# ucl-medical-genomics/hygeia

Hardware: AMD Instinct MI355X
Metric: CpG sites/sec through forward-backward; 28M CpG, K=6, 2 seeds, 1/2/4/8 GPUs (higher is better)
Workload: dtype f64; 1 GPU; C3 two_group 28000000 CpG (22 chromosomes, 100k segments + 5k buffers), 4+4 samples, K=6, M=50, B=25, 2 seeds in total, chains sharded over the GPUs (LPT); chains_per_rank=582, threads_per_chain=256, chains_per_cu_resident=3, global_sites_x_seeds=56000000, parallelism=chains over 1 rank(s) on 1 GPU(s)

## Files before the change

### hygeia_amd/_lib.py

```python
from __future__ import annotations

import ctypes as C
import math
import os

KMAX = 16
HERE = os.path.dirname(os.path.abspath(__file__))
LIB_PATH = os.path.join(HERE, "lib", "libhygeia_amd.so")

HYG_OK, HYG_EINVAL, HYG_ENUMERIC, HYG_EDEVICE, HYG_ENOMEM, HYG_EUNSUPPORTED = 0, -1, -2, -3, -4, -5
ERROR_NAMES = {0: "HYG_OK", -1: "HYG_EINVAL", -2: "HYG_ENUMERIC", -3: "HYG_EDEVICE", -4: "HYG_ENOMEM",
               -5: "HYG_EUNSUPPORTED"}


class HygError(RuntimeError):
    def __init__(self, code: int, msg: str):
        super().__init__(f"{ERROR_NAMES.get(code, code)}: {msg}")
        self.code = code


class TgParams(C.Structure):
    _fields_ = [
        ("n_regimes", C.c_int32),
        ("minimum_duration", C.c_int32),
# ... 70 lines not shown
        ("use_adam", C.c_int32),
        ("normalise_gradients", C.c_int32),
        ("n_steps_without_update", C.c_int32),
        ("_pad", C.c_int32),
        ("learning_rate_exponent", C.c_double),
        ("learning_rate_factor", C.c_double),
    ]


class SgChain(C.Structure):
    _fields_ = [
        ("site_begin", C.c_int64),
        ("n_sites", C.c_int32),
        ("_pad", C.c_int32),
        ("seed", C.c_uint64),
        ("chain_id", C.c_uint64),
        ("out_begin", C.c_int64),
    ]


EXPORTS = ("hyg_tg_params_default", "hyg_tg_model_create", "hyg_tg_model_destroy", "hyg_tg_num_particles",
           "hyg_tg_global_weights", "hyg_tg_backward_threads_per_chain", "hyg_tg_kernel_name",
           "hyg_tg_threads_per_chain", "hyg_tg_force_threads", "hyg_tg_set_tail_overlap", "hyg_tg_set_gather_window",
           "hyg_tg_device_cus",
           "hyg_tg_set_device_cus", "hyg_sg_force_key_drop", "hyg_tg_chains_per_cu", "hyg_tg_lds_bytes",
           "hyg_tg_emission", "hyg_tg_workspace_bytes", "hyg_tg_run_chains", "hyg_tg_run_chain_host",
           "hyg_tg_run_chains_host", "hyg_tg_models_compatible", "hyg_tg_workspace_bytes_multi",
           "hyg_tg_run_chains_multi", "hyg_tg_run_chains_host_multi", "hyg_tg_kernel_name_multi",
           "hyg_tg_filter_workspace_bytes", "hyg_tg_filter_workspace_bytes_multi", "hyg_tg_filter_chains",
           "hyg_tg_filter_chains_multi", "hyg_tg_filter_chains_host", "hyg_tg_filter_chains_host_multi",
           "hyg_tg_filter_kernel_name", "hyg_tg_filter_kernel_name_multi",
           "hyg_tg_trace_chains", "hyg_tg_trace_chains_multi", "hyg_tg_trace_chains_host",
           "hyg_tg_trace_chains_host_multi", "hyg_tg_trace_kernel_name", "hyg_tg_trace_kernel_name_multi",
           "hyg_device_count", "hyg_device_slot_acquire", "hyg_device_slot_release", "hyg_set_device",
           "hyg_get_device", "hyg_last_error", "hyg_version", "hyg_set_kernel_timing", "hyg_tg_last_kernel_ms",
           "hyg_sg_params_default", "hyg_sg_model_create", "hyg_sg_model_destroy", "hyg_sg_emission",
           "hyg_sg_workspace_bytes", "hyg_sg_run_chains", "hyg_sg_run_chain_host",
           "hyg_sg_pe_params_default", "hyg_sg_pe_theta_rows", "hyg_sg_pe_workspace_bytes", "hyg_sg_run_chains_pe",
           "hyg_sg_run_chain_host_pe", "hyg_sg_models_compatible", "hyg_sg_workspace_bytes_multi",
           "hyg_sg_pe_workspace_bytes_multi", "hyg_sg_run_chains_multi", "hyg_sg_run_chains_pe_multi",
           "hyg_sg_run_chains_host_multi", "hyg_bed_labels", "hyg_bed_format", "hyg_pre_collapse",
           "hyg_dmp_site_counts", "hyg_dmp_fdr", "hyg_dmp_weighted_fdr", "hyg_tg_posterior_counts")


class DmpGroup(C.Structure):

# ... 28 lines not shown
        _build.build()
    L = C.CDLL(path)
    vp, i32, i64, u64, sz = C.c_void_p, C.c_int32, C.c_int64, C.c_uint64, C.c_size_t
    L.hyg_tg_params_default.restype = None
    L.hyg_tg_params_default.argtypes = [C.POINTER(TgParams)]
    L.hyg_tg_model_create.restype = C.c_int
    L.hyg_tg_model_create.argtypes = [C.POINTER(TgParams), i32, i32, C.POINTER(vp)]
    L.hyg_tg_model_destroy.restype = None
    L.hyg_tg_model_destroy.argtypes = [vp]
    L.hyg_tg_num_particles.restype = i32
    L.hyg_tg_num_particles.argtypes = [vp]
    L.hyg_tg_global_weights.restype = i32
    L.hyg_tg_global_weights.argtypes = [vp]
    L.hyg_tg_threads_per_chain.restype = i32
    L.hyg_tg_threads_per_chain.argtypes = [vp, i32]
    L.hyg_tg_backward_threads_per_chain.restype = i32
    L.hyg_tg_backward_threads_per_chain.argtypes = [vp, i32]
    L.hyg_tg_force_threads.restype = C.c_int
    L.hyg_tg_force_threads.argtypes = [i32, i32]
    L.hyg_tg_set_tail_overlap.restype = C.c_int
    L.hyg_tg_set_tail_overlap.argtypes = [i32]
    L.hyg_tg_set_gather_window.restype = C.c_int
    L.hyg_tg_set_gather_window.argtypes = [i32]
    L.hyg_tg_device_cus.restype = i32
    L.hyg_tg_device_cus.argtypes = [i32]
    L.hyg_tg_set_device_cus.restype = C.c_int
    L.hyg_tg_set_device_cus.argtypes = [i32, i32]
    L.hyg_sg_force_key_drop.restype = C.c_int
    L.hyg_sg_force_key_drop.argtypes = [i32]
    L.hyg_tg_chains_per_cu.restype = i32
    L.hyg_tg_chains_per_cu.argtypes = [vp, i32]
    L.hyg_tg_lds_bytes.restype = sz
    L.hyg_tg_lds_bytes.argtypes = [vp, i32, i32]
    L.hyg_tg_kernel_name.restype = i32
    L.hyg_tg_kernel_name.argtypes = [vp, i32, i32, C.c_char_p, i32]
    L.hyg_tg_emission.restype = C.c_int
    L.hyg_tg_emission.argtypes = [vp, vp, vp, i32, vp, vp, i32, i64, vp, vp]
    L.hyg_tg_workspace_bytes.restype = sz
    L.hyg_tg_workspace_bytes.argtypes = [vp, i32, i64]
    L.hyg_tg_run_chains.restype = C.c_int
    L.hyg_tg_run_chains.argtypes = [vp, C.POINTER(TgChain), i32, vp, vp, sz, C.POINTER(TgOutputs), vp]
    L.hyg_tg_run_chain_host.restype = C.c_int
    L.hyg_tg_run_chain_host.argtypes = [vp, vp, vp, i32, vp, vp, i32, i32, u64, u64, vp, vp, vp, vp, vp, vp, vp]
    L.hyg_tg_run_chains_host.restype = C.c_int
    L.hyg_tg_run_chains_host.argtypes = [vp, vp, vp, i32, vp, vp, i32, i64, C.POINTER(TgChain), i32, i64,
                                         vp, vp, vp, vp, vp, vp, vp, vp]
# ... 162 lines not shown
```

### hygeia_amd/csrc/capi.cpp

```cpp
#include <hip/hip_runtime.h>
#include <fcntl.h>
#include <sys/file.h>
#include <unistd.h>

#include <algorithm>
#include <cerrno>
#include <cmath>
#include <cstdio>
#include <cstring>
#include <map>
#include <memory>
#include <mutex>
#include <string>
#include <vector>

#include "../../include/hyg_arith.h"
#include "../../include/hygeia_amd.h"
#include "../../include/hyg_sg_model.h"
#include "sg_common.h"
#include "tg_common.h"
#include "dmp_common.h"

namespace hyg {
int bed_launch_labels(const double* probs, int K, int64_t n, int8_t* label, double* score, void* stream);
// ... 365 lines not shown
int32_t hyg_tg_kernel_name(const hyg_tg_model* m, int32_t n_chains, int32_t backward, char* buf, int32_t len) {
  if (!m || len < 0) return fail(HYG_EINVAL, "null model or negative length");
  const char* name = nullptr;
  if (hyg::tg_kernel_name(m->c, n_chains, backward != 0, &name) != HYG_OK) return fail_unsupported_shape(m);
  const int32_t need = (int32_t)std::strlen(name) + 1;
  if (buf && len > 0) std::snprintf(buf, (size_t)len, "%s", name);
  return need;
}

int hyg_tg_force_threads(int32_t forward, int32_t backward) {
  const int rc = hyg::tg_force_threads(forward, backward);
  return rc == HYG_OK ? rc : fail(rc, "unsupported workgroup size");
}

int hyg_tg_set_tail_overlap(int32_t on) {
  hyg::tg_set_tail_overlap(on != 0);
  return HYG_OK;
}

int hyg_tg_set_gather_window(int32_t positions) {
  const int rc = hyg::tg_set_gather_window(positions);
  return rc == HYG_OK ? rc : fail(rc, "gather window out of [-1, 256]");
}

int32_t hyg_tg_device_cus(int32_t device) { return hyg::tg_device_cus(device); }

int hyg_tg_set_device_cus(int32_t device, int32_t cus) {
  const int rc = hyg::tg_set_device_cus(device, cus);
  return rc == HYG_OK ? rc : fail(rc, "device out of [0, 64) or negative CU count");
}

int hyg_sg_force_key_drop(int32_t bits) {
  const int rc = hyg::sg_force_key_drop(bits);
  return rc == HYG_OK ? rc : fail(rc, "key bits out of range [8, 60]");
}

int hyg_tg_emission(const hyg_tg_model* m, const uint16_t* meth_c, const uint16_t* tot_c, int32_t s_c,
                    const uint16_t* meth_k, const uint16_t* tot_k, int32_t s_k, int64_t n_sites, double* E,
                    void* stream) {
  if (!m) return fail(HYG_EINVAL, "null model");
  if (!m->on_device) return fail(HYG_EDEVICE, "no HIP device: hygeia_amd has no CPU fallback");
  if (!on_model_device(m->device)) return fail(HYG_EINVAL, "the current HIP device is not the model's device");
  if (s_c < 0 || s_k < 0 || n_sites < 0) return fail(HYG_EINVAL, "negative size");
  if (n_sites > 0 && (!E || (s_c && (!meth_c || !tot_c)) || (s_k && (!meth_k || !tot_k))))
    return fail(HYG_EINVAL, "null buffer");
  return launch_emission(m->dev(), m->c, meth_c, tot_c, s_c, meth_k, tot_k, s_k, n_sites, E, stream);
// ... 1408 lines not shown
```

### hygeia_amd/csrc/tg_common.h

```cpp
#pragma once

#include <stddef.h>
#include <stdint.h>

#include "../../include/hyg_model.h"

namespace hyg {

constexpr int kDefaultThreads = 256;
constexpr int kDefaultThreadsBwd = 256;
constexpr int kLowOccThreads = 512;
constexpr int kLowOccThreadsBwd = 768;
constexpr int kEBlock = 8;

struct ChainDev {
  int64_t site_begin;
  int64_t out_begin;
  int64_t ws_offset;
  uint64_t seed;
  uint64_t chain_id;
  int32_t T;
  int32_t pad;
  int64_t wg_offset;
};
// ... 35 lines not shown
int launch_chains_multi(const ModelDev* models_dev, const hyg_tg_consts& c, const ChainDev* chains_dev, int n_chains,
                        const double* E, uint8_t* ws, const hyg_tg_outputs& out, void* stream);
int launch_filter(const ModelDev& md, const hyg_tg_consts& c, const ChainDev* chains_dev, int n_chains,
                  const double* E, uint8_t* ws, const hyg_tg_outputs& out, void* stream);
int launch_filter_multi(const ModelDev* models_dev, const hyg_tg_consts& c, const ChainDev* chains_dev, int n_chains,
                        const double* E, uint8_t* ws, const hyg_tg_outputs& out, void* stream);
int launch_trace(const ModelDev& md, const hyg_tg_consts& c, const ChainDev* chains_dev, int n_chains, const double* E,
                 uint8_t* ws, const hyg_tg_outputs& out, const hyg_tg_trace& trace, void* stream);
int launch_trace_multi(const ModelDev* models_dev, const hyg_tg_consts& c, const ChainDev* chains_dev, int n_chains,
                       const double* E, uint8_t* ws, const hyg_tg_outputs& out, const hyg_tg_trace& trace,
                       void* stream);
void set_kernel_timing(bool on);
int last_kernel_ms(float* out3);
int tg_threads_per_chain(const hyg_tg_consts& c, int n_chains);
int tg_threads_per_chain_bwd(const hyg_tg_consts& c, int n_chains);
int tg_kernel_name(const hyg_tg_consts& c, int n_chains, bool backward, const char** name, bool multi = false);
int tg_filter_kernel_name(const hyg_tg_consts& c, int n_chains, const char** name, bool multi = false);
int tg_trace_kernel_name(const hyg_tg_consts& c, int n_chains, const char** name, bool multi = false);
size_t tg_trace_lds_bytes(const hyg_tg_consts& c, int n_chains);
int tg_force_threads(int fwd, int bwd);
int tg_resident_per_cu(const hyg_tg_consts& c, int n_chains);
void tg_set_tail_overlap(bool on);
int tg_set_gather_window(int positions);
int tg_device_cus(int dev);
int tg_set_device_cus(int dev, int cus);
size_t tg_layout_bytes(const hyg_tg_consts& c, int threads, bool backward);
bool backward_global_w(const hyg_tg_consts& c);
bool forward_global_w(const hyg_tg_consts& c);
size_t chain_scratch_bytes(const hyg_tg_consts& c);

}
```

### hygeia_amd/csrc/tg_kernels.hip

```cpp
#include <hip/hip_runtime.h>

#include <cstdio>
#include <cstdlib>
#include <atomic>
#include <mutex>
#include <vector>

#include "../../include/hyg_arith.h"
#include "tg_common.h"
#include "hyg_dev.h"

namespace hyg {

enum { MODE_KEEP = 0, MODE_OPTIMAL = 1, MODE_UNBIASED = 2, MODE_INIT = 3 };

#ifndef HYG_SERIAL_PRIO
#define HYG_SERIAL_PRIO 1
#endif
__device__ __forceinline__ void serial_begin() {
  if constexpr (HYG_SERIAL_PRIO > 0) __builtin_amdgcn_s_setprio(HYG_SERIAL_PRIO);
}
__device__ __forceinline__ void serial_end() {
  if constexpr (HYG_SERIAL_PRIO > 0) __builtin_amdgcn_s_setprio(0);
}


__device__ __forceinline__ uint64_t sort_key(float x, int idx) {
  uint32_t u = hyg_f32_bits(x);
  if (u == 0x80000000u) u = 0;
  const uint32_t ord = (u >> 31) ? ~u : (u | 0x80000000u);
  return ((uint64_t)(~ord) << 32) | (uint32_t)idx;
}
__device__ __forceinline__ float key_value(uint64_t k) {
  const uint32_t ord = ~(uint32_t)(k >> 32);
  const uint32_t u = (ord & 0x80000000u) ? (ord & 0x7fffffffu) : ~ord;
  return hyg_bits_f32(u);
}
__device__ __forceinline__ int key_index(uint64_t k) { return (int)(uint32_t)k; }

__device__ __forceinline__ int fdiv(int n, int d, float rd) {
  int q = (int)((float)n * rd);
  if (q * d > n) --q;
  if ((q + 1) * d <= n) ++q;
  return q;
}

template <int R>
// ... 208 lines not shown
#endif
#ifndef HYG_LR512
#define HYG_LR512 2
#endif
template <int NT>
constexpr int kLRof = NT >= 768 ? 2 : (NT >= 512 ? HYG_LR512 : HYG_LR256);
#ifndef HYG_SORT_WAVES
#define HYG_SORT_WAVES 4
#endif
#ifndef HYG_TSF1
#define HYG_TSF1 1
#endif
template <int NT>
constexpr int kSortWaves = (NT / 64 < HYG_SORT_WAVES) ? NT / 64 : HYG_SORT_WAVES;

struct Lay {
  uint32_t W, L, keys, bcnt, bpos, pre64, part, cp, pst, pw, phz, pf, ering, cl, parents, X, grp, gst, rb, xo, red,
      sh, uring, total;
  uint32_t bcnt_bytes;
  int npad, nkeys, nt;
  int topset_r;
  int lcap;
  int gather_w;
};

__host__ __device__ constexpr int bwd_list_doubles(int NT) {
  return (64 * 16 + 128 + 32) > 4 * (NT + 1) ? (64 * 16 + 128 + 32) : 4 * (NT + 1);
}

__host__ __device__ inline size_t fwd_keys_bytes(int Nmax, int NT) {
  size_t kb = sizeof(uint64_t) * (size_t)Nmax;
  if (kb < sizeof(hyg_u128) * (size_t)(NT + 1)) kb = sizeof(hyg_u128) * (size_t)(NT + 1);
  return kb;
}
__host__ __device__ inline size_t fwd_scratch_bytes(int Nmax, int NT) {
  return align_up(sizeof(double) * (size_t)Nmax, 16) + fwd_keys_bytes(Nmax, NT);
}

__host__ __device__ inline Lay make_layout(int K, int M, int B, int Nmax, int NT, bool backward, bool gw = false) {
  Lay l{};
  l.nt = NT;
  l.topset_r = 1;
  l.npad = Nmax;
  l.lcap = (backward && gw && bwd_list_doubles(NT) < Nmax) ? bwd_list_doubles(NT) : Nmax;
  size_t o = 0;
  if (!backward && gw) {
// ... 604 lines not shown
    for (int step = 32; step >= 1; step >>= 1) {
#pragma unroll
      for (int r = 0; r < NSW; ++r) pos[r] += (buf[64 * r + pos[r] + step - 1] < e) ? step : 0;
    }
    int rank = 0;
#pragma unroll
    for (int r = 0; r < NSW; ++r) rank += pos[r] + ((buf[64 * r + pos[r]] < e) ? 1 : 0);
    buf[64 * NSW + rank] = e;
  }
  lds_barrier();
  return sorter ? buf[64 * NSW + base] : e;
}

constexpr int bitonic_lds_stages(int n, int R) {
  int c = 0;
  for (int kk = 2; kk <= n; kk *= 2)
    for (int j = kk / 2; j >= 1; j /= 2) c += (j >= 64 * R) ? 1 : 0;
  return c;
}

template <int NT, int NSW, int R>
__device__ __forceinline__ int top_set_finish(uint64_t* srt, int nA, bool hasB, int N, int M, int cnt_fin, const hyg_u192& massB,
                              unsigned char* scr, int* parents, Shared& sh, const ConstLds& cl, unsigned char* red,
                              float Usys, unsigned long long* ph, bool timed) {
  static_assert(NSW <= NT / 64, "sorting waves");
  const int lane = lane_id();
  const bool sorter = (NSW == NT / 64) || wave_id() < NSW;
  const int base = (int)(threadIdx.x >> 6) * 64 * R + lane * R;
  uint64_t e[R];
  hyg_u192 f[R];
  hyg_u192 loc = hyg_u192_zero();
  if (sorter) {
#pragma unroll
    for (int r = 0; r < R; ++r) e[r] = (base + r < nA) ? srt[base + r] : ~0ull;
    int ib = 0;
    Bitonic<64 * NSW, R, 2, 1>::run(e, (uint64_t*)scr, ib);
    TPH(27);
#pragma unroll
    for (int r = 0; r < R; ++r) srt[base + r] = e[r];
#pragma unroll
    for (int r = 0; r < R; ++r) {
      const float m = hyg_expf(key_value(e[r]));
      f[r] = hyg_fix149f((base + r < nA) ? m : 0.0f);
      loc = hyg_u192_add(loc, f[r]);
    }
  } else {
    constexpr int nb = bitonic_lds_stages(64 * NSW * R, R);
#pragma unroll
    for (int i = 0; i < nb; ++i) lds_barrier();
#pragma unroll
    for (int r = 0; r < R; ++r) {
      e[r] = ~0ull;
      f[r] = hyg_u192_zero();
    }
  }
  hyg_u192 massA;
  const hyg_u192 ex = block_excl192<NT, false>(loc, red, &massA);
  hyg_u192* pre = (hyg_u192*)scr;
  const hyg_u192 total = hyg_u192_add(massA, massB);
  hyg_u192 run = ex;
  if (sorter) {
#pragma unroll
    for (int r = 0; r < R; ++r) {
      run = hyg_u192_add(run, f[r]);
      if (base + r < nA) pre[base + r] = run;
    }
  }
  lds_barrier();
  TPH(28);
  if (wave_id() == 0) {
    serial_begin();
    const int a = lane;
    const int cap = nA < M ? nA : M;
    float xk;
    if constexpr (R == 1) xk = key_value(e[0]);
    else xk = key_value(srt[lane < nA ? lane : 0]);
    const uint64_t capmask = (cap >= 64) ? ~0ull : ((1ull << cap) - 1ull);
    int flag = 0;
    float ca = 0.0f;
    hyg_u192 rva = hyg_u192_zero();
    if (a < M && a < N) {
      if (a <= nA) rva = hyg_u192_sub(total, a == 0 ? hyg_u192_zero() : pre[a - 1]);
      else if (hasB) flag = 1;
      const double rvd = hyg_u192_to_f64(rva);
      const float l2 = (rvd == 0.0) ? HYG_NINFF : (float)hyg_log(rvd);
      ca = cl.logMa[a] - l2;
    }
    TPH(30);
    int aa = 0, bb = -1, ovf = 0;
    while (aa != bb && aa < N && aa < M) {
      const float c = __builtin_bit_cast(float, __builtin_amdgcn_readlane(__builtin_bit_cast(int, ca), aa));
      int nxt = 0;
      if (hyg_isfinitef(c)) {
        nxt = (int)__builtin_popcountll(wave_ballot((float)(c + xk) > 0.0f) & capmask);
// ... 19 lines not shown
      const hyg_u192 tlast = rdlane192(tau, L > 0 ? L - 1 : 0);
      TPH(31);
      if (L > 0 && hasB && !hyg_u192_ge(massA, tlast)) {
        status = FAST_FALLBACK_REGEN;
      } else {
        if (lane < bb) parents[lane] = key_index(srt[lane]);
        if (lane < L) {
          int lo = bb, hi = nA - 1;
          while (lo < hi) {
            const int mid = (lo + hi) >> 1;
            if (hyg_u192_ge(pre[mid], tau)) hi = mid; else lo = mid + 1;
          }
          parents[bb + lane] = key_index(srt[lo]);
        }
        TPH(34);
      }
    }
    if (lane == 0) {
      sh.Kk = bb;
      sh.log_c = lc;
      sh.fast = status;
    }
    TPH(33);
    serial_end();
  }
  lds_barrier();
  TPH(29);
  return sh.fast;
}

__device__ __forceinline__ double u192_approx(const hyg_u192& a) {
  auto w = [](uint64_t x) { return fma((double)(uint32_t)(x >> 32), 0x1p32, (double)(uint32_t)x); };
  return fma(w(a.w2), 0x1p128, fma(w(a.w1), 0x1p64, w(a.w0)));
}

__device__ __forceinline__ int sys_count(const hyg_u192& v, const hyg_u192& R, double invR, int L, float U,
                                         const float* Ttab) {
  const double y = u192_approx(v) * invR;
  double jf = y * (double)L - (double)U;
  jf = jf < -1.0 ? -1.0 : (jf > (double)L ? (double)L : jf);
  const int j0 = (int)floor(jf);
  const double ylo = y * (1.0 - 0x1p-46), yhi = y * (1.0 + 0x1p-46);
  float T[2];
#pragma unroll
  for (int k = 0; k < 2; ++k) {
    const int j = j0 + k;
    T[k] = Ttab[j < 0 ? 0 : (j >= L ? L - 1 : j)];
// ... 51 lines not shown
template <int NT, int NSW>
__device__ __forceinline__ Ahead ahead_area(unsigned char* scr, size_t scr_bytes, int window) {
  constexpr size_t used = (tsf1_bytes<NSW>() + 15) / 16 * 16;
  constexpr size_t per = sizeof(uint64_t) + sizeof(double) + sizeof(Hz4);
  int n = scr_bytes > used ? (int)((scr_bytes - used) / per) : 0;
  n = n < window ? n : window;
  n = n < 64 * (NT / 64 - 1) ? n : 64 * (NT / 64 - 1);
  Ahead a;
  a.pos = (int*)scr;
  a.st = (uint64_t*)(scr + used);
  a.w = (double*)(scr + used + sizeof(uint64_t) * n);
  a.hz = (Hz4*)(scr + used + (sizeof(uint64_t) + sizeof(double)) * n);
  a.n = n > 0 ? n : 0;
  return a;
}

enum { FAST_DONE_AHEAD = 3 };

template <int NT, int NSW, bool SPLIT, class Anc>
__device__ __forceinline__ int top_set_finish1(uint64_t* srt, int nA, bool hasB, int N, int M, int cnt_fin,
                                               const hyg_u192& massB_in, unsigned char* scr, int* parents,
                                               Shared& sh, const ConstLds& cl, unsigned char* red, float Usys,
                                               const ListsB& lb, const Ahead& ah, Anc ancestor_of,
                                               unsigned long long* ph, bool timed) {
  static_assert(NSW <= NT / 64 && NSW <= 4, "sorting waves");
  constexpr int NW = NT / 64, NNS = NW - NSW;
  static_assert(!SPLIT || NNS >= NSW, "the outside masses need idle waves");
  const int lane = lane_id();
  const bool sorter = (NSW == NT / 64) || wave_id() < NSW;
  const int base = (int)(threadIdx.x >> 6) * 64 + lane;
  hyg_u192* preL = (hyg_u192*)(scr + 2 * 64 * NSW * sizeof(uint64_t));
  hyg_u192* wtot = (hyg_u192*)red;
  uint64_t e[1];
  hyg_u192 f = hyg_u192_zero(), inc = hyg_u192_zero();
  if (sorter) {
    e[0] = (base < nA) ? srt[base] : ~0ull - (uint64_t)base;
    e[0] = rank_sort_asc<NSW>(e[0], (uint64_t*)scr, true, []() {});
    TPH(27);
    srt[base] = e[0];
    const float m = hyg_expf(key_value(e[0]));
    f = hyg_fix149f((base < nA) ? m : 0.0f);
    inc = wave_incl192(f);
    preL[base] = inc;
    if (lane == 63) wtot[wave_id()] = inc;
  } else {
    static_assert(!SPLIT || NW <= 2 * NNS, "two lists per idle wave");
    hyg_u128 n128 = hyg_u128_zero();
    hyg_u192 m192 = hyg_u192_zero();
    const int v = wave_id() - NSW;
    if (SPLIT && hasB) list_mass(lb, v, n128, m192);
    (void)rank_sort_asc<NSW>(0, (uint64_t*)scr, false, [&]() {
      if (SPLIT && hasB && v + NNS < NW) list_mass(lb, v + NNS, n128, m192);
    });
    if (SPLIT && hasB) {
      if (lb.narrow) { m192.w0 = n128.lo; m192.w1 = n128.hi; m192.w2 = 0; }
      const hyg_u192 ws = wave_sum192(m192);
      if (lane == 0) lb.part_tot[v] = ws;
    }
    e[0] = ~0ull;
  }
  lds_barrier();
  TPH(28);
  if (wave_id() == 0) {
    serial_begin();
    hyg_u192 massA = hyg_u192_zero();
#pragma unroll
    for (int w = 0; w < NSW; ++w) massA = hyg_u192_add(massA, wtot[w]);
    hyg_u192 massB = massB_in;
    if (SPLIT && hasB) {
#pragma unroll
      for (int w = 0; w < NNS; ++w) massB = hyg_u192_add(massB, lb.part_tot[w]);
    }
    const hyg_u192 total = hyg_u192_add(massA, massB);
    const int a = lane;
    const float xk = key_value(e[0]);
    const int cap = nA < M ? nA : M;
    const uint64_t capmask = (cap >= 64) ? ~0ull : ((1ull << cap) - 1ull);
    int flag = 0;
    float ca = 0.0f;
    hyg_u192 rva = hyg_u192_zero();
    if (a < M && a < N) {
      if (a <= nA) rva = hyg_u192_sub(total, hyg_u192_sub(inc, f));
      else if (hasB) flag = 1;
      const double rvd = hyg_u192_to_f64(rva);
      const float l2 = (rvd == 0.0) ? HYG_NINFF : (float)hyg_log(rvd);
      ca = cl.logMa[a] - l2;
    }
// ... 43 lines not shown
          const int wp = pc >> 6;
          hyg_u192 C = preL[pc];
#pragma unroll
          for (int w = 1; w < NSW; ++w)
            if (wp == w) C = hyg_u192_add(C, wb[w]);
          const uint64_t key = srt[pc];
          const int cnt = sys_count(hyg_u192_sub(C, preK), Rr, invR, L, Usys, Ttab);
          const int cex = wave_shr1(cnt, cprev);
          for (int j = cex; j < cnt; ++j) parents[bb + j] = key_index(key);
          if (ah.n > 0)
            for (int j = cex; j < cnt; ++j) ah.pos[bb + j] = pc;
          cprev = __builtin_amdgcn_readlane(cnt, 63);
        }
        if (cprev < L) status = FAST_FALLBACK_REGEN;
      }
      TPH(34);
    }
    if (lane == 0) {
      sh.Kk = bb;
      sh.log_c = lc;
      sh.fast = (status == FAST_DONE && ah.n > 0) ? FAST_DONE_AHEAD : status;
    }
    TPH(33);
    serial_end();
  } else if (ah.n > 0) {
    const int p = (wave_id() - 1) * 64 + lane;
    if (p < ah.n && p < nA) {
      uint64_t s;
      double w;
      Hz4 h;
      ancestor_of(key_index(srt[p]), s, w, h);
      ah.st[p] = s;
      ah.w[p] = w;
      ah.hz[p] = h;
    }
  }
  lds_barrier();
  TPH(29);
  return sh.fast;
}

template <int NT, int NSW, class Anc>
__device__ __forceinline__ int top_set_resample(const double* W, int N, double mx, double logS, int* lst, int lb, int cw,
                                unsigned char* scr, size_t scr_bytes, uint64_t* srt, size_t srt_bytes,
                                const int* part_cnt, hyg_u192* part_tot, int* parents, Shared& sh,
                                const ConstLds& cl, unsigned char* red, int M, int cnt_fin, float Usys,
                                int rmax, const Ahead& ah, Anc ancestor_of, unsigned long long* ph, bool timed) {
  constexpr int NW = NT / 64;
  const int wv = wave_id(), lane = lane_id();
  static_assert(kNCut == 8 && NW * kNCut <= 128, "cutoff counts: one or two per lane");
  const int pc = (lane < NW * kNCut) ? part_cnt[lane] : 0;
  const int pc2 = (NW * kNCut > 64 && lane + 64 < NW * kNCut) ? part_cnt[lane + 64] : 0;
  int c = pc + pc2;
  c += (int)xshfl32<8>((uint32_t)c);
  c += (int)xshfl32<16>((uint32_t)c);
  c += (int)xshfl32<32>((uint32_t)c);
  const int np = (c <= 64 * NSW) ? 64 * NSW : 128 * NSW;
  const bool fits = lane < kNCut && c <= 64 * NSW * rmax && (size_t)np * sizeof(hyg_u192) <= scr_bytes &&
                    (size_t)np * 8 <= srt_bytes;
  const uint64_t fm = wave_ballot(fits);
  const int nL = __builtin_amdgcn_readlane(c, kNCut - 1);
  if (threadIdx.x == 0) sh.n_sig = nL;
  if (fm == 0) return FAST_FALLBACK;
  const int ks = 63 - __builtin_clzll(fm);
  const int nA = __builtin_amdgcn_readlane(c, ks);
  const bool hasB = nA < nL;
  const double cutx = (ks == kNCut - 1) ? HYG_NINF : -cut_below_top(ks);
  int off = 0;
  for (int w = 0; w < wv; ++w)
    off += __builtin_amdgcn_readlane(w < 8 ? pc : pc2, (w & 7) * kNCut + ks);
// ... 40 lines not shown
        const hyg_u128 f = hyg_fix149f_low128(outA[r] ? m : 0.0f);
        if (r & 1) nb2 = hyg_u128_add(nb2, f); else nb = hyg_u128_add(nb, f);
      }
    } else if (hasB) {
#pragma unroll
      for (int r = 0; r < kLR; ++r) {
        const float m = hyg_expf(lw[r]);
        const hyg_u192 f = hyg_fix149f(outA[r] ? m : 0.0f);
        if (r & 1) mb2 = hyg_u192_add(mb2, f); else mb = hyg_u192_add(mb, f);
      }
    }
  }
  if constexpr (kSplitB) {
    if (split) {
      lds_barrier();
      TPH(26);
      ListsB lbs;
      lbs.lst = lst;
      lbs.stride = ((N + NT - 1) / NT) * 64;
      lbs.part_cnt = part_cnt;
      lbs.part_tot = part_tot;
      lbs.narrow = ks >= kNarrowCut && 2 * ((N + NT - 1) / NT) <= kNarrowPerLane;
      return top_set_finish1<NT, NSW, kSplitB>(srt, nA, hasB, N, M, cnt_fin, hyg_u192_zero(), scr, parents, sh, cl,
                                               red, Usys, lbs, ah, ancestor_of, ph, timed);
    }
  }
  if (hasB) {
    if (narrow) {
      const hyg_u128 t = hyg_u128_add(nb, nb2);
      mb.w0 = t.lo; mb.w1 = t.hi; mb.w2 = 0;
    } else {
      mb = hyg_u192_add(mb, mb2);
    }
    const hyg_u192 ws = wave_sum192(mb);
    if (lane == 0) part_tot[wv] = ws;
  }
  lds_barrier();
  hyg_u192 massB = hyg_u192_zero();
  if (hasB) massB = sum_waves192<NW>(part_tot);
  TPH(26);
  if (nA <= 64 * NSW) {
#if HYG_TSF1
    if constexpr (NSW <= 4)
      if (scr_bytes >= tsf1_bytes<NSW>())
        return top_set_finish1<NT, NSW, false>(srt, nA, hasB, N, M, cnt_fin, massB, scr, parents, sh, cl, red, Usys,
                                               ListsB{}, ah, ancestor_of, ph, timed);
#endif
    return top_set_finish<NT, NSW, 1>(srt, nA, hasB, N, M, cnt_fin, massB, scr, parents, sh, cl, red, Usys, ph, timed);
  }
  return top_set_finish<NT, NSW, 2>(srt, nA, hasB, N, M, cnt_fin, massB, scr, parents, sh, cl, red, Usys, ph, timed);
}
#undef TPH

constexpr int kETile = 256;
#ifndef HYG_TG_FO_TU
__global__ void __launch_bounds__(kETile)
tg_emission_kernel(const double* __restrict__ lf, const double* __restrict__ lg, const double* __restrict__ cst,
                   int L, int K, const uint16_t* __restrict__ meth_c, const uint16_t* __restrict__ tot_c, int s_c,
                   const uint16_t* __restrict__ meth_k, const uint16_t* __restrict__ tot_k, int s_k, int64_t T,
                   double* __restrict__ E) {
  extern __shared__ __align__(16) unsigned char smem[];
  double* tile = (double*)smem;
  const int K2 = 2 * K;
  for (int64_t t0 = (int64_t)blockIdx.x * kETile; t0 < T; t0 += (int64_t)gridDim.x * kETile) {
    const int64_t t = t0 + threadIdx.x;
    if (t < T) {
      for (int g = 0; g < 2; ++g) {
        const int S = g ? s_k : s_c;
        const uint16_t* my = g ? meth_k + t * s_k : meth_c + t * s_c;
        const uint16_t* nt = g ? tot_k + t * s_k : tot_c + t * s_c;
        double e[HYG_KMAX];
        for (int r = 0; r < K; ++r) e[r] = 0.0;
        for (int s = 0; s < S; ++s) {
// ... 284 lines not shown
      StepScalars* s0 = (StepScalars*)rec0;
      s0->mode = MODE_INIT; s0->n_par = 0; s0->log_c = 0.0f; s0->r_ph = sh.r_ph; s0->lse = 0.0; s0->pad = 0.0;
    }
  }
  if (kURing && wave_id() == NT / 64 - 1 && lane_id() < kUR)
    uring[(1 + lane_id()) & (kUR - 1)] =
        hyg_u01f(hyg_rand64(ch.seed, ch.chain_id, HYG_RNG_SYSTEMATIC, (uint64_t)(1 + lane_id()), 0));
  lds_barrier();
  double mloc;
  int cloc;
  gen_weights_init<NT>(cl, K, sh.r_ph, erow(ering, 0, K2), W, &mloc, &cloc);
  if constexpr (GW) __syncthreads();
  int N = K * K, np_prev = 0, prev_mode = MODE_INIT;
  float prev_logc = 0.0f;
  double prev_lse = 0.0;
  double mx;
  int cnt;
  block_max_cnt<NT>(mloc, cloc, red, &mx, &cnt);

  Ahead ahead{};
  if constexpr (!GW && HYG_TSF1 && kSortWaves<NT> <= 4)
    ahead = ahead_area<NT, kSortWaves<NT>>(smem + lay.W, lay.bcnt - lay.W, lay_arg.gather_w);

  if (dbg && tid == 0) ph_acc[kPh - 1] = __builtin_amdgcn_s_memtime();
  for (int t = 1; t < T; ++t) {
    const uint64_t* pst = pst0 + cur * M;
    const double* pw = pw0 + cur * M;
    const Hz4* phz = phz0 + cur * M;
    auto ancestor_of = [&](int n, uint64_t& s, double& w, Hz4& h) {
      if (prev_mode == MODE_INIT) {
        s = init_state(K, n);
        const double2 hc = cl.hz1[0][hyg_st_rc(s)], hk = cl.hz1[1][hyg_st_rk(s)];
        h.lrc = hc.x; h.l1c = hc.y; h.lrk = hk.x; h.l1k = hk.y;
        const int i = n / K, j = n - (n / K) * K;
        const double* E0 = erow(ering, 0, K2);
        w = (E0[i] + E0[K + j]) + ((i == j) ? cl.lPc[sh.r_ph * K + i] : HYG_NINF);
      } else {
        const int sl = fdiv(n, np_prev, 1.0f / (float)np_prev);
        const int ao = n - sl * np_prev;
        const uint64_t anc = pst[ao];
        const Pf3 pfo = pf[ao];
        const Hz4 hzo = phz[ao];
        const double pao = pw[ao];
        s = tg_xi_hz_sel(cl, K, 1.0f / (float)K, anc, sl, pfo, &h);
        const double tr = tg_trans(cl, K, anc, s, hzo);
        const double* Ep = erow(ering, t - 1, K2);
        w = HYG_NINF;
        if (hyg_isfinite(tr)) {
// ... 111 lines not shown
    if (cnt <= M) {
      mode = MODE_KEEP;
      np = cnt;
      const int cs = (N + NT - 1) / NT;
      const int p0 = tid * cs, p1 = (p0 + cs < N) ? p0 + cs : N;
      int loc = 0;
      for (int n = p0; n < p1; ++n) loc += (W[n] > HYG_NINF);
      hyg_u128 v;
      v.lo = (uint64_t)loc;
      v.hi = 0;
      block_scan128<NT>(v, cp128, red);
      part_barrier<GW>();
      int o = (int)cp128[tid].lo;
      for (int n = p0; n < p1; ++n)
        if (W[n] > HYG_NINF) parents[o++] = n;
      PH(2);
      if (dbg && tid == 0) ph_acc[10]++;
    } else {
      PH(2);
      int fs = FAST_FALLBACK;
      if (topset)
        fs = top_set_resample<NT, kSortWaves<NT>>(W, N, mx, logS, lst, lst_base, lst_cnt, smem + lay.W, lay.bcnt - lay.W,
                                  (uint64_t*)(smem + lay.bcnt), lay.bcnt_bytes, part_cnt, part_tot, parents, sh, cl,
                                  red, M, cnt, Ucur, lay.topset_r, ahead, ancestor_of, ph_acc, dbg != nullptr);
      parked = fs == FAST_DONE_AHEAD;
      if (parked) fs = FAST_DONE;
      PH(20);
      if (fs != FAST_DONE) {
        if (fs == FAST_FALLBACK_REGEN) {
          if (prev_mode == MODE_INIT) {
            gen_weights_init<NT>(cl, K, sh.r_ph, erow(ering, t - 1, K2), W, &mloc, &cloc);
          } else {
            gen_weights<NT>(cl, K, I, np_prev, prev_mode, prev_logc, prev_lse, pst, pw, phz,
                            erow(ering, t - 1, K2), W, &mloc, &cloc);
          }
          lds_barrier();
        }
        optimal_resample<NT, GW>(W, (uint64_t*)W, N, mx, logS, sig_thresh, keys, bcnt, bpos, pre64, tau, parents,
                             sh, cl, red, M, cnt, ch.seed, ch.chain_id, t, Ucur, ph_acc, dbg != nullptr);
        if (dbg && tid == 0) ph_acc[21]++;
      }
      if (dbg && tid == 0) ph_acc[9] += sh.n_sig;
      PH(3);
      int Kk = sh.Kk;
      log_c = sh.log_c;
      if (Kk >= N) { Kk = N; log_c = HYG_NINFF; }
      np = M;
// ... 7 lines not shown
        } else {
          gen_weights<NT>(cl, K, I, np_prev, prev_mode, prev_logc, prev_lse, pst, pw, phz, erow(ering, t - 1, K2),
                          W, &mloc, &cloc);
        }
        part_barrier<GW>();
        auto logit = [&](int n) -> double {
          const double w = W[n];
          return (w > HYG_NINF) ? (double)(float)((w - mx) - logS) : HYG_NINF;
        };
        auto rnd = [&](int q) -> uint64_t {
          return hyg_rand64(ch.seed, ch.chain_id, HYG_RNG_MULTINOMIAL, (uint64_t)t, (uint64_t)q);
        };
        auto out = [&](int q, int n) { parents[q] = n; };
        auto all = [](int) { return true; };
        part_barrier<GW>();
        categorical_block<NT, GW>(N, lmax, logit, M, all, rnd, out, cp128, red);
      } else {
        mode = MODE_OPTIMAL;
        need_bar = fs != FAST_DONE;
      }
    }
    if (need_bar) part_barrier<GW>();
    PH(4);
    if (wave_id() == 0) serial_begin();
    StepScalars* rs = REC ? (StepScalars*)(rec0 + (size_t)t * rstride) : nullptr;
    uint64_t* rst = REC ? (uint64_t*)(rs + 1) : nullptr;
    double* rw = REC ? (double*)(rst + M) : nullptr;
    Pf3 pfa;
    uint64_t gs = 0;
    double gw = 0.0;
    Hz4 gh{};
    const bool have_pf = tid < np;
    if (have_pf) {
      const int a = tid;
      uint64_t s;
      double w;
      Hz4 h;
      const int pp = (parked && mode == MODE_OPTIMAL) ? ahead.pos[a] : ahead.n;
      if (pp < ahead.n) {
        s = ahead.st[pp];
        w = ahead.w[pp];
        h = ahead.hz[pp];
      } else {
        ancestor_of(parents[a], s, w, h);
      }
      gs = s;
      gw = w;
      gh = h;
      if constexpr (REC) {
        rst[a] = s;
        rw[a] = w;
      }
      pfa = prefetch_rows(md, K, s);
    }
    if constexpr (REC) {
      if (tid == 0) {
        rs->mode = mode; rs->n_par = np; rs->log_c = log_c; rs->r_ph = 0; rs->lse = lse; rs->pad = 0.0;
      }
    }
    if (wave_id() == 0) serial_end();
    if (kURing) {
      if (wave_id() == NT / 64 - 1 && (t & (kUR - 1)) == 0 && lane_id() < kUR)
        uring[(t + 1 + lane_id()) & (kUR - 1)] =
            hyg_u01f(hyg_rand64(ch.seed, ch.chain_id, HYG_RNG_SYSTEMATIC, (uint64_t)(t + 1 + lane_id()), 0));
    } else if (wave_id() == NT / 64 - 1) {
      const float un = hyg_u01f(hyg_rand64(ch.seed, ch.chain_id, HYG_RNG_SYSTEMATIC, (uint64_t)(t + 1), 0));
      if (lane_id() == 0) sh.Unext = un;
    }
    constexpr int EQ = (kEBlock * 2 * HYG_KMAX + NT - 1) / NT;
    double ebuf[EQ];
    int e_tot = 0;
    if (eload) {
      const int t0 = (t / kEBlock + 1) * kEBlock;
      const int rows = (T - t0) < kEBlock ? (T - t0) : kEBlock;
      e_tot = rows * K2;
#pragma unroll
      for (int q = 0; q < EQ; ++q) {
        const int i = tid + q * NT;
        ebuf[q] = (i < e_tot) ? Ech[(size_t)t0 * K2 + i] : 0.0;
      }
    }
    np_prev = np;
    prev_mode = mode;
// ... 695 lines not shown
  n = query_cus(dev);
  if (n > 0) g_cus[dev].store(n, std::memory_order_relaxed);
  return n;
}
int device_cus() {
  int dev = 0;
  if (hipGetDevice(&dev) != hipSuccess) return 256;
  const int n = cus_of(dev);
  return n > 0 ? n : 256;
}
int g_force_threads[2] = {0, 0};
bool valid_width(int x) { return x == 64 || x == 128 || x == 256 || x == 512 || x == 768; }
constexpr int kMaxGatherWindow = 256;
constexpr int kDefaultGatherWindow = 192;
std::atomic<int> g_gather_window{kDefaultGatherWindow};
}

int tg_set_gather_window(int positions) {
  if (positions < -1 || positions > kMaxGatherWindow) return HYG_EINVAL;
  g_gather_window.store(positions < 0 ? kDefaultGatherWindow : positions, std::memory_order_relaxed);
  return HYG_OK;
}

int tg_force_threads(int fwd, int bwd) {
  if ((fwd && !valid_width(fwd)) || (bwd && !valid_width(bwd))) return HYG_EINVAL;
  g_force_threads[0] = fwd;
  g_force_threads[1] = bwd;
  return HYG_OK;
}

int tg_device_cus(int dev) { return cus_of(dev); }
int tg_set_device_cus(int dev, int cus) {
  if (dev < 0 || dev >= kMaxDevices || cus < 0) return HYG_EINVAL;
  g_cus[dev].store(cus, std::memory_order_relaxed);
  return HYG_OK;
}

void set_kernel_timing(bool on) {
  std::lock_guard<std::mutex> lock(g_ev_mu);
  g_timing = on;
}

int last_kernel_ms(float* out3) {
  std::lock_guard<std::mutex> lock(g_ev_mu);
  for (int k = 0; k < 3; ++k) {
    out3[k] = -1.0f;
// ... 179 lines not shown
struct KernelPlan {
  int status;
  int nt;
  bool gw;
  Lay lay;
  const KernelRow* k;
  size_t lds;
};
static KernelPlan plan(bool backward, const hyg_tg_consts& c, int n_chains, bool mm = false, bool rec = true,
                       bool trc = false) {
  KernelPlan p{};
  p.nt = forward_global_w(c) ? 256 : pick_threads(backward, c, n_chains);
  const size_t more = trc ? trace_bins_extra(c.K) : 0;
  auto fits = [&](int nt) { return width_fits(backward, c, nt) && layout_at(backward, c, nt).total + more <= kCuLdsBytes; };
  if (!fits(p.nt)) p.nt = 256;
  p.gw = width_gw(backward, c, p.nt);
  p.lay = layout_at(backward, c, p.nt);
  p.lds = p.lay.total + more;
  p.status = fits(p.nt) ? HYG_OK : HYG_EUNSUPPORTED;
  static const int topset_r = tuning_int("HYG_TOPSET_R");
  if (!backward && (topset_r == 1 || topset_r == 2)) p.lay.topset_r = topset_r;
  static const char* window_env = tuning_env("HYG_GATHER_WINDOW");
  if (!backward) p.lay.gather_w = window_env ? atoi(window_env) : g_gather_window.load(std::memory_order_relaxed);
  static const bool phases = tuning_env("HYG_DEBUG_PHASES") != nullptr;
  p.k = find_row(backward, p.nt, shape_of(c), phases, p.gw, mm, rec, trc);
  return p;
}

int tg_threads_per_chain(const hyg_tg_consts& c, int n_chains) { return plan(false, c, n_chains).nt; }
int tg_threads_per_chain_bwd(const hyg_tg_consts& c, int n_chains) { return plan(true, c, n_chains).nt; }
int tg_kernel_name(const hyg_tg_consts& c, int n_chains, bool backward, const char** name, bool multi) {
  const KernelPlan p = plan(backward, c, n_chains, multi);
  *name = p.k->name;
  return p.status;
}
int tg_filter_kernel_name(const hyg_tg_consts& c, int n_chains, const char** name, bool multi) {
  const KernelPlan p = plan(false, c, n_chains, multi, false);
  *name = p.k->name;
  return p.status;
}
int tg_trace_kernel_name(const hyg_tg_consts& c, int n_chains, const char** name, bool multi) {
  const KernelPlan p = plan(false, c, n_chains, multi, false, true);
  *name = p.k->name;
  return p.status;
}
size_t tg_trace_lds_bytes(const hyg_tg_consts& c, int n_chains) { return plan(false, c, n_chains, false, false, true).lds; }
// ... 306 lines not shown
```

### include/hygeia_amd.h

```cpp
#ifndef HYGEIA_AMD_H
#define HYGEIA_AMD_H

#include <stddef.h>
#include <stdint.h>

#ifdef __cplusplus
extern "C" {
#endif

#define HYG_KMAX 16

#define HYG_OK 0
#define HYG_EINVAL (-1)
#define HYG_ENUMERIC (-2)
#define HYG_EDEVICE (-3)
#define HYG_ENOMEM (-4)
#define HYG_EUNSUPPORTED (-5)

typedef struct hyg_tg_params {
  int32_t n_regimes;
  int32_t minimum_duration;
  int32_t num_resampled_ancestors;
  int32_t num_samples_backward;
  int32_t optimal_resampling;
// ... 27 lines not shown
                        int32_t max_duration, hyg_tg_model** out);
void hyg_tg_model_destroy(hyg_tg_model* model);

int32_t hyg_tg_num_particles(const hyg_tg_model* model);

int32_t hyg_tg_global_weights(const hyg_tg_model* model);

int32_t hyg_tg_threads_per_chain(const hyg_tg_model* model, int32_t n_chains);

int32_t hyg_tg_backward_threads_per_chain(const hyg_tg_model* model, int32_t n_chains);

int32_t hyg_tg_chains_per_cu(const hyg_tg_model* model, int32_t n_chains);

size_t hyg_tg_lds_bytes(const hyg_tg_model* model, int32_t threads, int32_t backward);

int32_t hyg_tg_kernel_name(const hyg_tg_model* model, int32_t n_chains, int32_t backward, char* buf, int32_t len);

int hyg_tg_force_threads(int32_t forward, int32_t backward);

int hyg_tg_set_tail_overlap(int32_t on);

int hyg_tg_set_gather_window(int32_t positions);

int32_t hyg_tg_device_cus(int32_t device);

int hyg_tg_set_device_cus(int32_t device, int32_t cus);

int hyg_sg_force_key_drop(int32_t bits);

int hyg_tg_emission(const hyg_tg_model* model, const uint16_t* meth_ctrl, const uint16_t* tot_ctrl,
                    int32_t s_ctrl, const uint16_t* meth_case, const uint16_t* tot_case, int32_t s_case,
                    int64_t n_sites, double* emission, void* stream);

size_t hyg_tg_workspace_bytes(const hyg_tg_model* model, int32_t n_chains, int64_t total_steps);

typedef struct hyg_tg_outputs {
  int16_t* merged;
  int16_t* control;
  int16_t* kase;
  float* split_probs;
  float* regime_probs;
  double* log_z;
  double* final_log_weights;
  int32_t* status;
} hyg_tg_outputs;

// ... 226 lines not shown
```

Baseline: 22.77 million CpG-sites*seeds/s.

## Rotate wave scheduling priority across co-resident chains by realtime epoch

Adds a time-based rotation of the hardware wave priority (s_setprio) for the 256-thread forward kernel. The rotation is keyed on a slot taken from the HW_ID register modulo three, and every 8 steps each wave reads the realtime clock and picks a base priority from a 6-entry permutation table. Serial sections now raise priority relative to that base instead of a fixed level. The aim is fairer progress among the three chains resident per CU, so that no single chain straggles and lengthens the tail. In exchange it adds a clock read and priority switches inside the hot loop, and the HW_ID-derived slot may not match which chains actually share a SIMD.

```diff
diff --git a/hygeia_amd/_lib.py b/hygeia_amd/_lib.py
--- a/hygeia_amd/_lib.py
+++ b/hygeia_amd/_lib.py
@@ -116,6 +116,7 @@
 EXPORTS = ("hyg_tg_params_default", "hyg_tg_model_create", "hyg_tg_model_destroy", "hyg_tg_num_particles",
            "hyg_tg_global_weights", "hyg_tg_backward_threads_per_chain", "hyg_tg_kernel_name",
            "hyg_tg_threads_per_chain", "hyg_tg_force_threads", "hyg_tg_set_tail_overlap", "hyg_tg_set_gather_window",
+           "hyg_tg_set_priority_rotation", "hyg_tg_priority_base", "hyg_tg_priority_epoch_ticks",
            "hyg_tg_device_cus",
            "hyg_tg_set_device_cus", "hyg_sg_force_key_drop", "hyg_tg_chains_per_cu", "hyg_tg_lds_bytes",
            "hyg_tg_emission", "hyg_tg_workspace_bytes", "hyg_tg_run_chains", "hyg_tg_run_chain_host",
@@ -190,6 +191,12 @@
     L.hyg_tg_set_tail_overlap.argtypes = [i32]
     L.hyg_tg_set_gather_window.restype = C.c_int
     L.hyg_tg_set_gather_window.argtypes = [i32]
+    L.hyg_tg_set_priority_rotation.restype = C.c_int
+    L.hyg_tg_set_priority_rotation.argtypes = [i32]
+    L.hyg_tg_priority_base.restype = i32
+    L.hyg_tg_priority_base.argtypes = [u64, i32]
+    L.hyg_tg_priority_epoch_ticks.restype = i32
+    L.hyg_tg_priority_epoch_ticks.argtypes = []
     L.hyg_tg_device_cus.restype = i32
     L.hyg_tg_device_cus.argtypes = [i32]
     L.hyg_tg_set_device_cus.restype = C.c_int
diff --git a/hygeia_amd/csrc/capi.cpp b/hygeia_amd/csrc/capi.cpp
--- a/hygeia_amd/csrc/capi.cpp
+++ b/hygeia_amd/csrc/capi.cpp
@@ -411,6 +411,15 @@
   const int rc = hyg::tg_set_gather_window(positions);
   return rc == HYG_OK ? rc : fail(rc, "gather window out of [-1, 256]");
 }
+
+int hyg_tg_set_priority_rotation(int32_t on) {
+  hyg::tg_set_priority_rotation(on != 0);
+  return HYG_OK;
+}
+
+int32_t hyg_tg_priority_base(uint64_t ticks, int32_t slot) { return hyg::tg_priority_base(ticks, slot); }
+
+int32_t hyg_tg_priority_epoch_ticks(void) { return hyg::tg_priority_epoch_ticks(); }
 
 int32_t hyg_tg_device_cus(int32_t device) { return hyg::tg_device_cus(device); }
 
diff --git a/hygeia_amd/csrc/tg_common.h b/hygeia_amd/csrc/tg_common.h
--- a/hygeia_amd/csrc/tg_common.h
+++ b/hygeia_amd/csrc/tg_common.h
@@ -81,6 +81,9 @@
 int tg_resident_per_cu(const hyg_tg_consts& c, int n_chains);
 void tg_set_tail_overlap(bool on);
 int tg_set_gather_window(int positions);
+void tg_set_priority_rotation(bool on);
+int tg_priority_base(unsigned long long ticks, int slot);
+int tg_priority_epoch_ticks();
 int tg_device_cus(int dev);
 int tg_set_device_cus(int dev, int cus);
 size_t tg_layout_bytes(const hyg_tg_consts& c, int threads, bool backward);
diff --git a/hygeia_amd/csrc/tg_kernels.hip b/hygeia_amd/csrc/tg_kernels.hip
--- a/hygeia_amd/csrc/tg_kernels.hip
+++ b/hygeia_amd/csrc/tg_kernels.hip
@@ -17,12 +17,46 @@
 #ifndef HYG_SERIAL_PRIO
 #define HYG_SERIAL_PRIO 1
 #endif
-__device__ __forceinline__ void serial_begin() {
-  if constexpr (HYG_SERIAL_PRIO > 0) __builtin_amdgcn_s_setprio(HYG_SERIAL_PRIO);
-}
-__device__ __forceinline__ void serial_end() {
-  if constexpr (HYG_SERIAL_PRIO > 0) __builtin_amdgcn_s_setprio(0);
-}
+__device__ __forceinline__ void set_prio(int p) {
+  switch (p) {
+    case 0: __builtin_amdgcn_s_setprio(0); break;
+    case 1: __builtin_amdgcn_s_setprio(1); break;
+    case 2: __builtin_amdgcn_s_setprio(2); break;
+    default: __builtin_amdgcn_s_setprio(3); break;
+  }
+}
+#ifndef HYG_SERIAL_TOP
+#define HYG_SERIAL_TOP 0
+#endif
+__device__ __forceinline__ void serial_begin(int pb = 0) {
+  if constexpr (HYG_SERIAL_PRIO > 0) set_prio((HYG_SERIAL_TOP && (pb & 4)) ? 3 : (pb & 3) + HYG_SERIAL_PRIO);
+}
+__device__ __forceinline__ void serial_end(int pb = 0) {
+  if constexpr (HYG_SERIAL_PRIO > 0) set_prio(pb & 3);
+}
+
+#ifndef HYG_PRIO_ROT
+#define HYG_PRIO_ROT 1
+#endif
+constexpr int kPrioEpochShift = 15;
+constexpr int kPrioEvery = 8;
+__device__ __forceinline__ int wave_slot3() {
+  unsigned s;
+  asm volatile("s_getreg_b32 %0, hwreg(HW_REG_HW_ID, 0, 4)" : "=s"(s));
+  return (int)(s % 3u);
+}
+constexpr unsigned long long prio_orders() {
+  const int o[6][3] = {{0, 1, 2}, {1, 2, 0}, {2, 0, 1}, {0, 2, 1}, {2, 1, 0}, {1, 0, 2}};
+  unsigned long long v = 0;
+  for (int e = 0; e < 6; ++e)
+    for (int s = 0; s < 3; ++s) v |= (unsigned long long)o[e][s] << (2 * (3 * e + s));
+  return v;
+}
+__host__ __device__ constexpr int prio_base_at(unsigned long long ticks, int slot3) {
+  const unsigned e = (unsigned)(ticks >> kPrioEpochShift) % 6u;
+  return (int)((prio_orders() >> (2 * (3 * e + (unsigned)slot3))) & 3ull);
+}
+__device__ __forceinline__ int prio_base(int slot3) { return prio_base_at(__builtin_amdgcn_s_memrealtime(), slot3); }
 
 
 __device__ __forceinline__ uint64_t sort_key(float x, int idx) {
@@ -277,6 +311,7 @@
   int topset_r;
   int lcap;
   int gather_w;
+  int prio_rot;
 };
 
 __host__ __device__ constexpr int bwd_list_doubles(int NT) {
@@ -927,7 +962,7 @@
 template <int NT, int NSW, int R>
 __device__ __forceinline__ int top_set_finish(uint64_t* srt, int nA, bool hasB, int N, int M, int cnt_fin, const hyg_u192& massB,
                               unsigned char* scr, int* parents, Shared& sh, const ConstLds& cl, unsigned char* red,
-                              float Usys, unsigned long long* ph, bool timed) {
+                              float Usys, unsigned long long* ph, bool timed, int pb) {
   static_assert(NSW <= NT / 64, "sorting waves");
   const int lane = lane_id();
   const bool sorter = (NSW == NT / 64) || wave_id() < NSW;
@@ -974,7 +1009,7 @@
   lds_barrier();
   TPH(28);
   if (wave_id() == 0) {
-    serial_begin();
+    serial_begin(pb);
     const int a = lane;
     const int cap = nA < M ? nA : M;
     float xk;
@@ -1040,7 +1075,7 @@
       sh.fast = status;
     }
     TPH(33);
-    serial_end();
+    serial_end(pb);
   }
   lds_barrier();
   TPH(29);
@@ -1138,7 +1173,7 @@
                                                const hyg_u192& massB_in, unsigned char* scr, int* parents,
                                                Shared& sh, const ConstLds& cl, unsigned char* red, float Usys,
                                                const ListsB& lb, const Ahead& ah, Anc ancestor_of,
-                                               unsigned long long* ph, bool timed) {
+                                               unsigned long long* ph, bool timed, int pb) {
   static_assert(NSW <= NT / 64 && NSW <= 4, "sorting waves");
   constexpr int NW = NT / 64, NNS = NW - NSW;
   static_assert(!SPLIT || NNS >= NSW, "the outside masses need idle waves");
@@ -1178,7 +1213,7 @@
   lds_barrier();
   TPH(28);
   if (wave_id() == 0) {
-    serial_begin();
+    serial_begin(pb);
     hyg_u192 massA = hyg_u192_zero();
 #pragma unroll
     for (int w = 0; w < NSW; ++w) massA = hyg_u192_add(massA, wtot[w]);
@@ -1268,7 +1303,7 @@
       sh.fast = (status == FAST_DONE && ah.n > 0) ? FAST_DONE_AHEAD : status;
     }
     TPH(33);
-    serial_end();
+    serial_end(pb);
   } else if (ah.n > 0) {
     const int p = (wave_id() - 1) * 64 + lane;
     if (p < ah.n && p < nA) {
@@ -1291,7 +1326,7 @@
                                 unsigned char* scr, size_t scr_bytes, uint64_t* srt, size_t srt_bytes,
                                 const int* part_cnt, hyg_u192* part_tot, int* parents, Shared& sh,
                                 const ConstLds& cl, unsigned char* red, int M, int cnt_fin, float Usys,
-                                int rmax, const Ahead& ah, Anc ancestor_of, unsigned long long* ph, bool timed) {
+                                int rmax, const Ahead& ah, Anc ancestor_of, unsigned long long* ph, bool timed, int pb) {
   constexpr int NW = NT / 64;
   const int wv = wave_id(), lane = lane_id();
   static_assert(kNCut == 8 && NW * kNCut <= 128, "cutoff counts: one or two per lane");
@@ -1378,7 +1413,7 @@
       lbs.part_tot = part_tot;
       lbs.narrow = ks >= kNarrowCut && 2 * ((N + NT - 1) / NT) <= kNarrowPerLane;
       return top_set_finish1<NT, NSW, kSplitB>(srt, nA, hasB, N, M, cnt_fin, hyg_u192_zero(), scr, parents, sh, cl,
-                                               red, Usys, lbs, ah, ancestor_of, ph, timed);
+                                               red, Usys, lbs, ah, ancestor_of, ph, timed, pb);
     }
   }
   if (hasB) {
@@ -1400,11 +1435,11 @@
     if constexpr (NSW <= 4)
       if (scr_bytes >= tsf1_bytes<NSW>())
         return top_set_finish1<NT, NSW, false>(srt, nA, hasB, N, M, cnt_fin, massB, scr, parents, sh, cl, red, Usys,
-                                               ListsB{}, ah, ancestor_of, ph, timed);
+                                               ListsB{}, ah, ancestor_of, ph, timed, pb);
 #endif
-    return top_set_finish<NT, NSW, 1>(srt, nA, hasB, N, M, cnt_fin, massB, scr, parents, sh, cl, red, Usys, ph, timed);
-  }
-  return top_set_finish<NT, NSW, 2>(srt, nA, hasB, N, M, cnt_fin, massB, scr, parents, sh, cl, red, Usys, ph, timed);
+    return top_set_finish<NT, NSW, 1>(srt, nA, hasB, N, M, cnt_fin, massB, scr, parents, sh, cl, red, Usys, ph, timed, pb);
+  }
+  return top_set_finish<NT, NSW, 2>(srt, nA, hasB, N, M, cnt_fin, massB, scr, parents, sh, cl, red, Usys, ph, timed, pb);
 }
 #undef TPH
 
@@ -1735,8 +1770,20 @@
   if constexpr (!GW && HYG_TSF1 && kSortWaves<NT> <= 4)
     ahead = ahead_area<NT, kSortWaves<NT>>(smem + lay.W, lay.bcnt - lay.W, lay_arg.gather_w);
 
+  constexpr bool kRot = HYG_PRIO_ROT && NT == 256;
+  const bool rot = kRot && lay_arg.prio_rot != 0;
+  const int slot3 = kRot ? wave_slot3() : 0;
+  int pb = 0;
+
   if (dbg && tid == 0) ph_acc[kPh - 1] = __builtin_amdgcn_s_memtime();
   for (int t = 1; t < T; ++t) {
+    if constexpr (kRot) {
+      if (rot && (t & (kPrioEvery - 1)) == 1) {
+        pb = __builtin_amdgcn_readfirstlane(prio_base(slot3));
+        set_prio(pb);
+        if constexpr (HYG_SERIAL_TOP) pb |= 4;
+      }
+    }
     const uint64_t* pst = pst0 + cur * M;
     const double* pw = pw0 + cur * M;
     const Hz4* phz = phz0 + cur * M;
@@ -1894,7 +1941,7 @@
       if (topset)
         fs = top_set_resample<NT, kSortWaves<NT>>(W, N, mx, logS, lst, lst_base, lst_cnt, smem + lay.W, lay.bcnt - lay.W,
                                   (uint64_t*)(smem + lay.bcnt), lay.bcnt_bytes, part_cnt, part_tot, parents, sh, cl,
-                                  red, M, cnt, Ucur, lay.topset_r, ahead, ancestor_of, ph_acc, dbg != nullptr);
+                                  red, M, cnt, Ucur, lay.topset_r, ahead, ancestor_of, ph_acc, dbg != nullptr, pb);
       parked = fs == FAST_DONE_AHEAD;
       if (parked) fs = FAST_DONE;
       PH(20);
@@ -1948,7 +1995,7 @@
     }
     if (need_bar) part_barrier<GW>();
     PH(4);
-    if (wave_id() == 0) serial_begin();
+    if (wave_id() == 0) serial_begin(pb);
     StepScalars* rs = REC ? (StepScalars*)(rec0 + (size_t)t * rstride) : nullptr;
     uint64_t* rst = REC ? (uint64_t*)(rs + 1) : nullptr;
     double* rw = REC ? (double*)(rst + M) : nullptr;
@@ -1984,7 +2031,7 @@
         rs->mode = mode; rs->n_par = np; rs->log_c = log_c; rs->r_ph = 0; rs->lse = lse; rs->pad = 0.0;
       }
     }
-    if (wave_id() == 0) serial_end();
+    if (wave_id() == 0) serial_end(pb);
     if (kURing) {
       if (wave_id() == NT / 64 - 1 && (t & (kUR - 1)) == 0 && lane_id() < kUR)
         uring[(t + 1 + lane_id()) & (kUR - 1)] =
@@ -2726,6 +2773,13 @@
   return HYG_OK;
 }
 
+std::atomic<int> g_prio_rot{1};
+void tg_set_priority_rotation(bool on) { g_prio_rot.store(on ? 1 : 0, std::memory_order_relaxed); }
+int tg_priority_base(unsigned long long ticks, int slot) {
+  return slot < 0 ? -1 : prio_base_at(ticks, slot % 3);
+}
+int tg_priority_epoch_ticks() { return 1 << kPrioEpochShift; }
+
 int tg_force_threads(int fwd, int bwd) {
   if ((fwd && !valid_width(fwd)) || (bwd && !valid_width(bwd))) return HYG_EINVAL;
   g_force_threads[0] = fwd;
@@ -2951,6 +3005,7 @@
   if (!backward && (topset_r == 1 || topset_r == 2)) p.lay.topset_r = topset_r;
   static const char* window_env = tuning_env("HYG_GATHER_WINDOW");
   if (!backward) p.lay.gather_w = window_env ? atoi(window_env) : g_gather_window.load(std::memory_order_relaxed);
+  if (!backward) p.lay.prio_rot = g_prio_rot.load(std::memory_order_relaxed);
   static const bool phases = tuning_env("HYG_DEBUG_PHASES") != nullptr;
   p.k = find_row(backward, p.nt, shape_of(c), phases, p.gw, mm, rec, trc);
   return p;
diff --git a/include/hygeia_amd.h b/include/hygeia_amd.h
--- a/include/hygeia_amd.h
+++ b/include/hygeia_amd.h
@@ -73,6 +73,11 @@
 
 int hyg_tg_set_gather_window(int32_t positions);
 
+int hyg_tg_set_priority_rotation(int32_t on);
+
+int32_t hyg_tg_priority_base(uint64_t ticks, int32_t slot);
+int32_t hyg_tg_priority_epoch_ticks(void);
+
 int32_t hyg_tg_device_cus(int32_t device);
 
 int hyg_tg_set_device_cus(int32_t device, int32_t cus);
```

Result: faster. 23.90 million CpG-sites*seeds/s (median of 6 runs) (+5.0%).
